# jzhoulab/orca

Hardware: AMD Instinct MI355X
Metric: Mb of sequence encoded+decoded per second (32Mb H1-ESC-shaped model, both strands, 6 levels) (higher is better)
Workload: dtype f16x2 | Encoder Conv1d stages 1-7: f16x2 = fp32 emulated as 2 x fp16 split operands, 3 MFMA products, fp32 accumulate (22 significant operand bits); Decoder / Decoder_1m Conv2d: f16x2 = fp32 emulated as 2 x fp16 split operands, 3 MFMA products, fp32 accumulate (22 significant operand bits); Encoder2; 1 GPU; H1-ESC 32Mb model forward, single random 32Mb sequence, fp32-class (f16x2 split operands on the 16-bit matrix cores, see dtype; parity vs the reference's fp32 in `parity` with --full), both strands (genomepredict-equivalent, 1 model): Encoder+Encoder2+6 Decoder+Decoder_1m per strand; sequence_bp=32000000, strands=2, levels=6, weights=synthetic seed 0, input=1 byte/base packed sequence in HBM, both strands read from it, parallelism=single GPU

## Files before the change

### include/orca_hip.h

```cpp
#ifndef ORCA_HIP_H
#define ORCA_HIP_H

#include <stddef.h>
#include <stdint.h>

#ifdef __cplusplus
extern "C" {
#endif

#define ORCA_OK 0
#define ORCA_EINVAL (-1)
#define ORCA_EHIP (-2)
#define ORCA_ENOMEM (-3)
#define ORCA_ENODEV (-4)

#define ORCA_ABI_VERSION 1

typedef struct orca_ctx orca_ctx;
typedef struct orca_net orca_net;

enum orca_net_kind {
  ORCA_NET_ENCODER = 1,
  ORCA_NET_ENCODER2 = 2,
  ORCA_NET_ENCODER3 = 3,
// ... 33 lines not shown
  int32_t ksize;
} orca_kernel_time;
int orca_ctx_set_timing(orca_ctx* ctx, int enable);
int orca_ctx_get_timing(orca_ctx* ctx, orca_kernel_time* out, int max, int* n);

int orca_ctx_launch_counts(orca_ctx* ctx, int64_t* counts4);

int orca_net_create(orca_ctx* ctx, int kind, const orca_conv_desc* convs, int n_convs,
                    int upsample_mode, orca_net** out);
int orca_net_free(orca_net* net);

#define ORCA_PRECISION_F32 0
#define ORCA_PRECISION_BF16 1
#define ORCA_PRECISION_BF16X2 2
#define ORCA_PRECISION_BF16X3 3
#define ORCA_PRECISION_F16X2 4
#define ORCA_PRECISION_F16 5
int orca_net_set_precision(orca_net* net, int precision);
#define ORCA_ENCODER_FORM_DEFAULT 0
#define ORCA_ENCODER_FORM_STORED_RESIDUAL 1
#define ORCA_ENCODER_FORM_LCONV1_ONLY 2
#define ORCA_ENCODER_FORM_TWO_CONV 3
int orca_net_set_encoder_form(orca_net* net, int form);
int orca_ctx_take_overflow(orca_ctx* ctx, int* flag);


int orca_encoder_forward(orca_ctx* ctx, orca_net* net, const float* x, int64_t sx_b, int64_t sx_c,
                         int64_t sx_l, int B, int64_t L, int64_t bin_lo, int64_t bin_hi, float* out,
                         int64_t so_b, int64_t so_c, int64_t chunk_bp);

int orca_pack_sequence(orca_ctx* ctx, const float* x, int64_t sx_c, int64_t sx_l, int64_t L, uint8_t* codes_out, int* packable);
int orca_encoder_forward_codes(orca_ctx* ctx, orca_net* net, const uint8_t* codes, int64_t sc_b, int reverse, int B, int64_t L,
                               int64_t bin_lo, int64_t bin_hi, float* out, int64_t so_b, int64_t so_c, int64_t chunk_bp);
int orca_encoder_forward_codes_window(orca_ctx* ctx, orca_net* net, const uint8_t* codes, int64_t sc_b, int64_t win_origin,
                                      int64_t win_len, int reverse, int B, int64_t L, int64_t bin_lo, int64_t bin_hi,
                                      float* out, int64_t so_b, int64_t so_c, int64_t chunk_bp);
int orca_encoder_forward_2bit(orca_ctx* ctx, orca_net* net, const uint8_t* two, const uint8_t* nmask, int64_t start, int reverse, int64_t L,
                              int64_t bin_lo, int64_t bin_hi, float* out, int64_t so_c, int64_t chunk_bp);

int64_t orca_p16_plane_units(int64_t n);
int orca_encoder_stage3_planes(orca_ctx* ctx, orca_net* net, const uint8_t* codes, int64_t L, int reverse, float* planes, int64_t plane_units);
int orca_p16_pool5_into(orca_ctx* ctx, const float* src, int64_t src_units, int64_t src_pos0, float* dst, int64_t dst_units, int64_t dst_pos0, int64_t count);
int orca_encoder_front_snippet(orca_ctx* ctx, orca_net* net, const uint8_t* codes, int64_t L, int reverse, int64_t base0, int64_t nbases, int64_t skip,
                               int64_t count, float* dst, int64_t dst_units, int64_t dst_pos0);
int orca_encoder_back(orca_ctx* ctx, orca_net* net, const float* s4, int64_t s4_units, int64_t n4, float* out, int64_t so_c);
int orca_encoder_stage4_rows(orca_ctx* ctx, orca_net* net, const float* s4, int64_t s4_units, int64_t n4, float* rows);
// ... 71 lines not shown
#define ORCA_COMM_ID_BYTES 128
int orca_comm_unique_id(void* id128_host);
int orca_comm_init_rank(orca_ctx* ctx, int nranks, int rank, const void* id128_host, orca_comm** out);
int orca_comm_destroy(orca_comm* comm);
int orca_allgather(orca_ctx* ctx, orca_comm* comm, const float* send, float* recv, size_t count);

int orca_pointwise1d_forward(orca_ctx* ctx, const float* w_dev, const float* bias_dev, int cout, int cin, const float* x,
                             int64_t x_bs, int64_t ldx, float* y, int64_t y_bs, int64_t ldy, int B, int64_t n, int act);

int orca_conv1d_forward(orca_ctx* ctx, const orca_conv_desc* conv, const float* x, int64_t x_bs, int64_t ldx,
                        float* y, int64_t y_bs, int64_t ldy, const float* r1, const float* r2, int B, int64_t n,
                        int relu, int tile);
int orca_conv1d_nlc_forward(orca_ctx* ctx, const orca_conv_desc* conv, int precision, const float* x, float* y,
                            const float* r1, int B, int64_t n, int relu);
int orca_conv1d_p16_forward(orca_ctx* ctx, const orca_conv_desc* conv, const float* x, float* y, const float* r1,
                            int64_t n, int relu, int out_mode);
int orca_conv1d_b16_forward(orca_ctx* ctx, const orca_conv_desc* conv, const float* x, float* y, const float* r1,
                            int64_t n, int relu, int out_mode);
int orca_conv2d_forward(orca_ctx* ctx, const orca_conv_desc* conv, const float* x, float* y, const float* r,
                        int B, int n, int relu);
int orca_conv2d_m16_forward(orca_ctx* ctx, const orca_conv_desc* conv, int precision, const float* x, float* y,
                            const float* r, int B, int n, int relu);
int orca_conv2d_dblock_forward(orca_ctx* ctx, const orca_conv_desc* convs, int precision, const float* x, float* y, int B, int n);
int orca_maxpool1d_forward(orca_ctx* ctx, const float* x, int64_t ldx, float* y, int64_t ldy, int64_t rows,
                           int64_t n_out, int k);

#ifdef __cplusplus
}
#endif
#endif
```

### orca_amd/_lib.py

```python
import ctypes
import os
from ctypes import POINTER, c_char_p, c_int, c_int32, c_int64, c_size_t, c_void_p

_HERE = os.path.dirname(os.path.abspath(__file__))
LIB_PATH = os.path.join(_HERE, "csrc", "liborca_hip.so")

ORCA_NET_ENCODER, ORCA_NET_ENCODER2, ORCA_NET_ENCODER3, ORCA_NET_DECODER, ORCA_NET_DECODER_1M, ORCA_NET_ENCODER2B = 1, 2, 3, 4, 5, 6
ORCA_UPSAMPLE_NEAREST, ORCA_UPSAMPLE_BILINEAR = 0, 1
PRECISIONS = {"f32": 0, "bf16": 1, "bf16x2": 2, "bf16x3": 3, "f16x2": 4, "f16": 5}
ENCODER_FORMS = {"default": 0, "stored_residual": 1, "lconv1_only": 2, "two_conv": 3}


class OrcaHipError(RuntimeError):
    pass


class ConvDesc(ctypes.Structure):
    _fields_ = [("weight_host", c_void_p), ("bias_host", c_void_p), ("cout", c_int32), ("cin", c_int32),
                ("ksize", c_int32), ("dilation", c_int32)]


class KernelTime(ctypes.Structure):
    _fields_ = [("cout", c_int32), ("cin", c_int32), ("tile", c_int32), ("batch", c_int32), ("n", c_int64),
                ("ms", ctypes.c_float), ("ksize", c_int32)]


SIGNATURES = {
    "orca_abi_version": (c_int, []),
    "orca_last_error": (c_char_p, []),
    "orca_device_count": (c_int, []),
    "orca_ctx_create": (c_int, [c_int, c_void_p, POINTER(c_void_p)]),
    "orca_ctx_destroy": (c_int, [c_void_p]),
    "orca_ctx_set_stream": (c_int, [c_void_p, c_void_p]),
    "orca_ctx_workspace_bytes": (c_int, [c_void_p, POINTER(c_size_t)]),
    "orca_ctx_release_workspace": (c_int, [c_void_p]),
    "orca_ctx_take_overflow": (c_int, [c_void_p, POINTER(c_int)]),
    "orca_ctx_set_timing": (c_int, [c_void_p, c_int]),
    "orca_ctx_get_timing": (c_int, [c_void_p, POINTER(KernelTime), c_int, POINTER(c_int)]),
    "orca_ctx_launch_counts": (c_int, [c_void_p, POINTER(ctypes.c_int64)]),
    "orca_net_create": (c_int, [c_void_p, c_int, POINTER(ConvDesc), c_int, c_int, POINTER(c_void_p)]),
    "orca_net_free": (c_int, [c_void_p]),
    "orca_net_set_precision": (c_int, [c_void_p, c_int]),
    "orca_net_set_encoder_form": (c_int, [c_void_p, c_int]),
    "orca_encoder_forward": (c_int, [c_void_p, c_void_p, c_void_p, c_int64, c_int64, c_int64, c_int, c_int64, c_int64,
                                     c_int64, c_void_p, c_int64, c_int64, c_int64]),
    "orca_p16_plane_units": (c_int64, [c_int64]),
    "orca_encoder_stage3_planes": (c_int, [c_void_p, c_void_p, c_void_p, c_int64, c_int, c_void_p, c_int64]),
    "orca_p16_pool5_into": (c_int, [c_void_p, c_void_p, c_int64, c_int64, c_void_p, c_int64, c_int64, c_int64]),
    "orca_encoder_front_snippet": (c_int, [c_void_p, c_void_p, c_void_p, c_int64, c_int, c_int64, c_int64, c_int64, c_int64, c_void_p, c_int64, c_int64]),
    "orca_encoder_back": (c_int, [c_void_p, c_void_p, c_void_p, c_int64, c_int64, c_void_p, c_int64]),
    "orca_encoder_stage4_rows": (c_int, [c_void_p, c_void_p, c_void_p, c_int64, c_int64, c_void_p]),
    "orca_rows_pool5_into": (c_int, [c_void_p, c_void_p, c_int64, c_int64, c_void_p, c_int64, c_int64, c_int64]),
    "orca_encoder_front4_snippet": (c_int, [c_void_p, c_void_p, c_void_p, c_int64, c_int, c_int64, c_int64, c_int64, c_int64, c_void_p, c_int64, c_int64]),
    "orca_encoder_front4_ranges": (c_int, [c_void_p, c_void_p, c_void_p, c_int64, c_int, c_int, POINTER(ctypes.c_int64), c_void_p, c_int64]),
    "orca_encoder_back5": (c_int, [c_void_p, c_void_p, c_void_p, c_int64, c_void_p, c_int64]),
    "orca_screen_edit_codes": (c_int, [c_void_p, c_void_p, c_int64, c_void_p, c_int, c_void_p, c_int64, c_void_p, c_int64]),
    "orca_screen_splice_rows": (c_int, [c_void_p, c_void_p, c_int64, c_void_p, c_int64, c_void_p, c_int, c_void_p]),
    "orca_encoder_back5_batch": (c_int, [c_void_p, c_void_p, c_void_p, c_int, c_int64, c_void_p, c_int64, c_int64]),
    "orca_screen_scores": (c_int, [c_void_p, c_void_p, c_int64, c_void_p, c_int, c_int, c_void_p, c_void_p, c_void_p]),
    "orca_screen_edit_codes_multi": (c_int, [c_void_p, c_void_p, c_int64, c_void_p, c_void_p, c_int, c_void_p, c_void_p, c_int64, c_void_p, c_int64, c_void_p,
                                             c_int64]),
    "orca_screen_splice_rows_multi": (c_int, [c_void_p, c_void_p, c_int64, c_void_p, c_int64, c_void_p, c_void_p, c_int64, c_void_p, c_void_p, c_int, c_void_p]),
    "orca_screen_region_scores": (c_int, [c_void_p, c_void_p, c_int64, c_void_p, c_int, c_int, c_void_p, c_void_p, c_int, c_void_p, c_void_p]),
    "orca_screen_assemble_codes": (c_int, [c_void_p, c_void_p, c_int64, c_void_p, c_void_p, c_int, c_void_p, c_void_p, c_int64, c_void_p, c_int64, c_void_p,
                                           c_int64]),
    "orca_screen_gather_rows": (c_int, [c_void_p, c_void_p, c_int64, c_void_p, c_int64, c_void_p, c_void_p, c_void_p, c_int, c_void_p, c_void_p, c_int64, c_void_p,
# ... 14 lines not shown
    "orca_decoder_forward_rows": (c_int, [c_void_p, c_void_p, POINTER(c_void_p), c_int64, c_int64, POINTER(c_void_p), c_int64, c_int64, c_int64,
                                          POINTER(c_void_p), c_int64, c_int64, c_int64, c_int, c_int, c_void_p, c_int]),
    "orca_decoder1m_forward_rows": (c_int, [c_void_p, c_void_p, POINTER(c_void_p), c_int64, c_int64, c_int, c_int, c_void_p, c_int]),
    "orca_net_num_targets": (c_int, [c_void_p, POINTER(c_int)]),
    "orca_decoder1m_forward": (c_int, [c_void_p, c_void_p, c_void_p, c_int64, c_int64, c_int64, c_int, c_int, c_void_p, c_int]),
    "orca_decoder_probe": (c_int, [c_void_p, c_void_p, c_void_p, c_int64, c_int64, c_int64, c_void_p, c_int64, c_int64, c_int64, c_int64, c_void_p,
                                   c_int64, c_int64, c_int64, c_int64, c_int, c_int, c_int, c_int, c_void_p]),
    "orca_strand_merge": (c_int, [c_void_p, c_void_p, c_void_p, c_void_p, c_int]),
    "orca_block_mean_f64": (c_int, [c_void_p, c_void_p, c_int64, c_int64, c_int64, c_int, c_int, c_void_p, c_void_p, c_int]),
    "orca_adaptive_coarsegrain": (c_int, [c_void_p, c_void_p, c_void_p, c_int64, c_int, ctypes.c_float, c_int, c_int, c_void_p, c_int64]),
    "orca_genome_unpack_2bit": (c_int, [c_void_p, c_void_p, c_void_p, c_int64, c_int64, c_void_p]),
    "orca_comm_unique_id": (c_int, [c_void_p]),
    "orca_comm_init_rank": (c_int, [c_void_p, c_int, c_int, c_void_p, POINTER(c_void_p)]),
    "orca_comm_destroy": (c_int, [c_void_p]),
    "orca_allgather": (c_int, [c_void_p, c_void_p, c_void_p, c_void_p, c_size_t]),
    "orca_conv1d_forward": (c_int, [c_void_p, POINTER(ConvDesc), c_void_p, c_int64, c_int64, c_void_p, c_int64, c_int64,
                                    c_void_p, c_void_p, c_int, c_int64, c_int, c_int]),
    "orca_conv1d_nlc_forward": (c_int, [c_void_p, POINTER(ConvDesc), c_int, c_void_p, c_void_p, c_void_p, c_int, c_int64, c_int]),
    "orca_conv1d_p16_forward": (c_int, [c_void_p, POINTER(ConvDesc), c_void_p, c_void_p, c_void_p, c_int64, c_int, c_int]),
    "orca_conv1d_b16_forward": (c_int, [c_void_p, POINTER(ConvDesc), c_void_p, c_void_p, c_void_p, c_int64, c_int, c_int]),
    "orca_conv2d_forward": (c_int, [c_void_p, POINTER(ConvDesc), c_void_p, c_void_p, c_void_p, c_int, c_int, c_int]),
    "orca_conv2d_m16_forward": (c_int, [c_void_p, POINTER(ConvDesc), c_int, c_void_p, c_void_p, c_void_p, c_int, c_int, c_int]),
    "orca_conv2d_dblock_forward": (c_int, [c_void_p, POINTER(ConvDesc), c_int, c_void_p, c_void_p, c_int, c_int]),
    "orca_maxpool1d_forward": (c_int, [c_void_p, c_void_p, c_int64, c_void_p, c_int64, c_int64, c_int64, c_int]),
    "orca_pointwise1d_forward": (c_int, [c_void_p, c_void_p, c_void_p, c_int, c_int, c_void_p, c_int64, c_int64, c_void_p, c_int64,
                                          c_int64, c_int, c_int64, c_int]),
}

_lib = None


def load():
    global _lib
    if _lib is not None:
        return _lib
    if not os.path.exists(LIB_PATH):
        raise OrcaHipError(
            f"{LIB_PATH} not found: the HIP extension is not built. Run `make -C orca_amd/csrc` "
            "(or `python -c 'import __graft_entry__ as g; g.build()'`). There is no CPU fallback.")
    import torch
    lib = ctypes.CDLL(LIB_PATH)
    for name, (res, args) in SIGNATURES.items():
        fn = getattr(lib, name)
        fn.restype = res
        fn.argtypes = args
    if lib.orca_abi_version() != 1:
# ... 10 lines not shown
```

### orca_amd/csrc/conv2d_dblock.h

```cpp
#pragma once
#include "conv2d_m16.h"

struct DBlockArgs {
  f32x4* cur;
  const void* w[4];
  const float* bias[4];
  long bs;
  int H, W, dil;
  unsigned* flag;
};

#ifndef DBLOCK_STORE_WT
#define DBLOCK_STORE_WT 0
#endif
__device__ __forceinline__ void db_store_unit(u32x4_t* p, const u32x4_t& v) {
#if DBLOCK_STORE_WT
  m16_store_unit(p, v);
#else
  *p = v;
#endif
}

template <int NS, int DT, int ABL = 0>
__global__ __launch_bounds__(512, NS == 1 ? 4 : 2) void conv2d_dblock_kernel(DBlockArgs a) {
// ... 213 lines not shown
        unit_.x = h0_; unit_.y = h1_; unit_.z = l0_; unit_.w = l1_;
        if (pvalid) db_store_unit(reinterpret_cast<u32x4_t*>(cur) + m16_plane(h * 4 + q, g, NS, H) + poff, unit_);
      }
    if (pvalid && vmax > 65504.f) overflow = true;
  } else {
#pragma unroll
    for (int h = 0; h < 2; ++h)
#pragma unroll
      for (int qp = 0; qp < 2; ++qp) {
        const f32x4 v0 = acc4(h, 2 * qp, 128 + h * 32, true) + get_A(h * 4 + 2 * qp);
        const f32x4 v1 = acc4(h, 2 * qp + 1, 128 + h * 32, true) + get_A(h * 4 + 2 * qp + 1);
        if (DT == 1) vmax = p16_vmax3_abs(p16_vmax3_abs(p16_vmax3_abs(p16_vmax3_abs(vmax, v0.x, v0.y), v0.z, v0.w), v1.x, v1.y), v1.z, v1.w);
        unsigned a0_ = m16_pk2<DT>(v0.x, v0.y), a1_ = m16_pk2<DT>(v0.z, v0.w), b0_ = m16_pk2<DT>(v1.x, v1.y), b1_ = m16_pk2<DT>(v1.z, v1.w);
        p16_swap32(a0_, b0_);
        p16_swap32(a1_, b1_);
        u32x4_t unit_;
        unit_.x = a0_; unit_.y = a1_; unit_.z = b0_; unit_.w = b1_;
        if (pvalid) db_store_unit(reinterpret_cast<u32x4_t*>(cur) + m16_plane(h * 4 + 2 * qp + g, 0, NS, H) + poff, unit_);
      }
    if (DT == 1 && pvalid && vmax > 65504.f) overflow = true;
  }
  if (DT == 1 && overflow && a.flag) *a.flag = 1u;
}
```

### orca_amd/csrc/orca_core.hip

```cpp
#include "orca_internal.h"

static thread_local std::string g_err;

int fail(int code, const char* fmt, ...) {
  char buf[1024];
  va_list ap;
  va_start(ap, fmt);
  vsnprintf(buf, sizeof buf, fmt, ap);
  va_end(ap);
  g_err = buf;
  return code;
}

int ws_ensure(orca_ctx* ctx, size_t bytes) {
  ctx->ws_off = 0;
  if (ctx->ws_used && ctx->ws_stream != ctx->stream) HIPCHECK(hipStreamSynchronize(ctx->ws_stream));
  ctx->ws_stream = ctx->stream;
  ctx->ws_used = true;
  if (bytes <= ctx->ws_bytes) return ORCA_OK;
  const size_t step = bytes >= (size_t(1) << 30) ? (size_t(1) << 30) : (size_t(64) << 20);
  bytes = (bytes + step - 1) / step * step;
  if (ctx->ws) {
    HIPCHECK(hipStreamSynchronize(ctx->stream));
    HIPCHECK(hipFree(ctx->ws));
// ... 517 lines not shown
  *out = net;
  return ORCA_OK;
}

extern "C" int orca_net_set_precision(orca_net* net, int precision) {
  if (!net) return fail(ORCA_EINVAL, "net is NULL");
  if (precision < ORCA_PRECISION_F32 || precision > ORCA_PRECISION_F16) return fail(ORCA_EINVAL, "unknown precision %d", precision);
  const bool dec = net->kind == ORCA_NET_DECODER || net->kind == ORCA_NET_DECODER_1M;
  const bool unet = net->kind == ORCA_NET_ENCODER2 || net->kind == ORCA_NET_ENCODER3 || net->kind == ORCA_NET_ENCODER2B;
  if (precision != ORCA_PRECISION_F32 && !(((net->kind == ORCA_NET_ENCODER || unet) && precision != ORCA_PRECISION_F16) ||
                                           (dec && (precision == ORCA_PRECISION_F16X2 || precision == ORCA_PRECISION_BF16 || precision == ORCA_PRECISION_F16))))
    return fail(ORCA_EINVAL, "precision %d is not implemented for net kind %d", precision, net->kind);
  net->precision = precision;
  return ORCA_OK;
}

extern "C" int orca_net_set_encoder_form(orca_net* net, int form) {
  if (!net || net->kind != ORCA_NET_ENCODER) return fail(ORCA_EINVAL, "orca_net_set_encoder_form: not an Encoder net");
  if (form < ORCA_ENCODER_FORM_DEFAULT || form > ORCA_ENCODER_FORM_TWO_CONV) return fail(ORCA_EINVAL, "orca_net_set_encoder_form: form %d unknown", form);
  net->enc_form = form;
  return ORCA_OK;
}

extern "C" int orca_net_free(orca_net* net) {
  if (!net) return ORCA_OK;
  if (net->ctx) (void)hipSetDevice(net->ctx->device);
  for (auto& L : net->convs) free_layer(L);
  if (net->d_first_w) (void)hipFree(net->d_first_w);
  if (net->d_first_w16) (void)hipFree(net->d_first_w16);
  if (net->d_first_tab) (void)hipFree(net->d_first_tab);
  if (net->d_sep) (void)hipFree(net->d_sep);
  if (net->d_l1_w16) (void)hipFree(net->d_l1_w16);
  if (net->d_l1_bias) (void)hipFree(net->d_l1_bias);
  if (net->d_c1a_w16) (void)hipFree(net->d_c1a_w16);
  if (net->d_c1a_bias) (void)hipFree(net->d_c1a_bias);
  if (net->d_l1_f32) (void)hipFree(net->d_l1_f32);
  if (net->d_c1a_f32) (void)hipFree(net->d_c1a_f32);
  if (net->d_l1_bias32) (void)hipFree(net->d_l1_bias32);
  if (net->d_c1a_bias32) (void)hipFree(net->d_c1a_bias32);
  for (auto& L : net->comp) free_layer(L);
  delete net;
  return ORCA_OK;
}


extern "C" int orca_net_num_targets(orca_net* net, int* num_2d) {
// ... 6 lines not shown
```

### orca_amd/csrc/orca_decoder.hip

```cpp
#include "orca_internal.h"

#include "conv2d_m16.h"
#include "conv2d_m16q.h"
#include "conv2d_dblock.h"
#include "misc_kernels.h"
#include "coarsegrain.h"

int launch_conv2d(orca_ctx* ctx, const ConvLayer& L, const float* x, long x_bs, float* y, long y_bs,
                         const float* r, long r_bs, int B, int n, int relu) {
  if (L.ksize != 3) return fail(ORCA_EINVAL, "launch_conv2d on a non-3x3 layer");
  Conv2dArgs a;
  a.x = x; a.w = L.d_w; a.bias = L.d_bias; a.y = y; a.r = r;
  a.x_bs = x_bs; a.y_bs = y_bs; a.r_bs = r_bs; a.H = n; a.W = n; a.dil = L.dil; a.nchunks = L.nchunks; a.relu = relu;
  dim3 grid((unsigned)n, (unsigned)B);
  if (L.cout == 64) hipLaunchKernelGGL((conv2d_3x3_kernel<64>), grid, dim3(512), 0, ctx->stream, a);
  else hipLaunchKernelGGL((conv2d_3x3_kernel<32>), grid, dim3(512), 0, ctx->stream, a);
  LAUNCHCHECK("conv2d_3x3_kernel");
  return ORCA_OK;
}

int launch_conv2d_m16(orca_ctx* ctx, const ConvLayer& L, const f32x4* x, long x_bs, int x_oct, f32x4* y, long y_bs, int y_oct,
                             const f32x4* r, long r_bs, int B, int n, int relu, int mode, int chunk0, int nchunks_,
                             const float* tab, long tab_bs) {
  const bool bf16 = mode == 1;
// ... 147 lines not shown
        C2(L[7], Bf, sz64, 8, Df, sz64, 8, Cf, sz64, 1);
      } else {
        C2(pairs[0], A, szA, oA, T, sz32, 4, nullptr, 0, 0);
        C2(pairs[1], T, sz32, 4, Cf, sz64, 8, nullptr, 0, 0);
        C2(pairs[2], Cf, sz64, 8, T, sz32, 4, nullptr, 0, 1);
        C2(pairs[3], T, sz32, 4, Df, sz64, 8, Cf, sz64, 1);
      }
    } else {
      pairs = L; npairs = 19;
      C2(pairs[0], IN, szIN, oIN, T, sz32, 4, nullptr, 0, 0);
      C2(pairs[1], T, sz32, 4, Cf, sz64, 8, nullptr, 0, 0);
      C2(pairs[2], Cf, sz64, 8, T, sz32, 4, nullptr, 0, 1);
      C2(pairs[3], T, sz32, 4, Df, sz64, 8, Cf, sz64, 1);
    }
    f32x4* cur = Df;
    f32x4* oth = Cf;
    for (int i = 1; i < npairs; ++i) {
      PROBE(3 + i - 1, cur, sz64);
      const ConvLayer* p = pairs + 4 * i;
      const int dil = p[0].dil;
      if (dil >= 16) {
        if (!(dil == 16 || dil == 32 || dil == 64) || p[1].dil != dil || p[2].dil != dil || p[3].dil != dil)
          return fail(ORCA_EINVAL, "decoder block %d: dilation %d unsupported", i, dil);
        DBlockArgs da;
        da.cur = cur; da.bs = sz64; da.H = n; da.W = n; da.dil = dil; da.flag = ctx->d_flag;
        for (int k = 0; k < 4; ++k) {
          if (!bf16 && !p[k].f16_ok) return fail(ORCA_EINVAL, "layer weights exceed the fp16 range");
          da.w[k] = bf16 ? p[k].d_wb16p : p[k].d_wf16;
          da.bias[k] = p[k].d_bias;
        }
        hipLaunchKernelGGL((conv2d_dblock_kernel<NS, DT>), dim3(256, (unsigned)nb), dim3(512), 0, ctx->stream, da);
        LAUNCHCHECK("conv2d_dblock_kernel");
        continue;
      }
      C2(p[0], cur, sz64, 8, T, sz32, 4, nullptr, 0, 0);
      C2(p[1], T, sz32, 4, oth, sz64, 8, cur, sz64, 0);
      C2(p[2], oth, sz64, 8, T, sz32, 4, nullptr, 0, 1);
      C2(p[3], T, sz32, 4, cur, sz64, 8, oth, sz64, 1);
    }
#undef C2
    PROBE(3 + npairs - 1, cur, sz64);
#undef PROBE
    const ConvLayer& fa = net->convs[net->convs.size() - 2];
    const ConvLayer& fb = net->convs[net->convs.size() - 1];
    FinalArgs fa_;
    fa_.cur = reinterpret_cast<const float*>(cur); fa_.w1 = fa.d_w; fa_.b1 = fa.d_bias; fa_.w2 = fb.d_w; fa_.b2 = fb.d_bias; fa_.out = out + (size_t)b0 * nt2 * n * n;
// ... 218 lines not shown
```

### orca_amd/csrc/orca_internal.h

```cpp
#pragma once
#include <hip/hip_runtime.h>

#include <cstdarg>
#include <cstdint>
#include <cstdio>
#include <cstdlib>
#include <cstring>
#include <string>
#include <vector>

#include "conv_kernels.h"
#include "orca_hip.h"

int fail(int code, const char* fmt, ...) __attribute__((format(printf, 2, 3)));

#define HIPCHECK(expr)                                                                          \
  do {                                                                                          \
    hipError_t _e = (expr);                                                                     \
    if (_e != hipSuccess) return fail(ORCA_EHIP, "%s failed: %s (%s:%d)", #expr, hipGetErrorString(_e), __FILE__, __LINE__); \
  } while (0)

#define LAUNCHCHECK(name)                                                                        \
  do {                                                                                          \
    hipError_t _e = hipGetLastError();                                                          \
// ... 38 lines not shown
  return rc;
}

#ifndef ORCA_MAX_TARGETS
#define ORCA_MAX_TARGETS 8
#endif
#define ORCA_EDGE_SLAB (40 * 128)

struct ConvLayer {
  int cin = 0, cout = 0, ksize = 0, dil = 1;
  int kc = 8, nchunks = 0;
  float* d_w = nullptr;
  float* d_bias = nullptr;
  void* d_wb16 = nullptr;
  void* d_wf16 = nullptr;
  void* d_wb16p = nullptr;
  bool f16_ok = true;
};

struct orca_net {
  orca_ctx* ctx = nullptr;
  int kind = 0;
  int precision = ORCA_PRECISION_F32;
  int enc_form = ORCA_ENCODER_FORM_DEFAULT;
  float* d_first_w = nullptr;
  void* d_first_w16 = nullptr;
  float* d_first_tab = nullptr;
  int upsample_mode = ORCA_UPSAMPLE_BILINEAR;
  int num_2d = 1;
  float* d_sep = nullptr;
  void* d_l1_w16 = nullptr;
  float* d_l1_bias = nullptr;
  void* d_c1a_w16 = nullptr;
  float* d_c1a_bias = nullptr;
  float* d_l1_f32 = nullptr;
  float* d_c1a_f32 = nullptr;
  float* d_l1_bias32 = nullptr;
  float* d_c1a_bias32 = nullptr;
  ConvLayer comp[3];
  std::vector<ConvLayer> convs;
};

int make_layer(const orca_conv_desc& d, ConvLayer* out);
int make_layer17(int cin, int cout, const std::vector<double>& w17, const std::vector<double>& b17, ConvLayer* out);
void compose_pair(const orca_conv_desc& c1, const orca_conv_desc& c2, std::vector<double>* w17, std::vector<double>* b17);
void free_layer(ConvLayer& L);
// ... 50 lines not shown
```

### orca_amd/csrc/orca_test_entries.hip

```cpp
#include "orca_internal.h"

#include "conv_p16.h"
#include "conv2d_m16.h"
#include "conv2d_dblock.h"
#include "misc_kernels.h"

extern "C" int orca_conv1d_forward(orca_ctx* ctx, const orca_conv_desc* conv, const float* x, int64_t x_bs, int64_t ldx, float* y,
                                   int64_t y_bs, int64_t ldy, const float* r1, const float* r2, int B, int64_t n, int relu,
                                   int tile) {
  if (!ctx || !conv || !x || !y) return fail(ORCA_EINVAL, "orca_conv1d_forward: NULL argument");
  HIPCHECK(hipSetDevice(ctx->device));
  ConvLayer L;
  ORCA_TRY(make_layer(*conv, &L));
  int rc = launch_conv1d(ctx, L, x, x_bs, ldx, y, y_bs, ldy, r1, r2, B, n, relu, tile);
  (void)hipStreamSynchronize(ctx->stream);
  free_layer(L);
  return rc;
}

extern "C" int orca_conv1d_nlc_forward(orca_ctx* ctx, const orca_conv_desc* conv, int precision, const float* x, float* y,
                                       const float* r1, int B, int64_t n, int relu) {
  if (!ctx || !conv || !x || !y) return fail(ORCA_EINVAL, "orca_conv1d_nlc_forward: NULL argument");
  if (precision < ORCA_PRECISION_BF16 || precision > ORCA_PRECISION_F16X2) return fail(ORCA_EINVAL, "precision %d unsupported here", precision);
  HIPCHECK(hipSetDevice(ctx->device));
// ... 160 lines not shown
  if (!(d == 16 || d == 32 || d == 64)) return fail(ORCA_EINVAL, "orca_conv2d_dblock_forward: dilation %d (16, 32 or 64)", d);
  for (int k = 0; k < 4; ++k) {
    const int cin = k & 1 ? 32 : 64, cout = k & 1 ? 64 : 32;
    if (convs[k].ksize != 3 || convs[k].cin != cin || convs[k].cout != cout || convs[k].dilation != d)
      return fail(ORCA_EINVAL, "orca_conv2d_dblock_forward: conv %d must be 3x3, %d -> %d, dilation %d", k, cin, cout, d);
  }
  HIPCHECK(hipSetDevice(ctx->device));
  ConvLayer L[4];
  int rc = ORCA_OK;
  for (int k = 0; k < 4 && rc == ORCA_OK; ++k) {
    rc = make_layer(convs[k], &L[k]);
    if (rc == ORCA_OK && precision != ORCA_PRECISION_BF16 && !L[k].f16_ok) rc = fail(ORCA_EINVAL, "layer weights exceed the fp16 range");
  }
  if (rc == ORCA_OK) {
    if (precision == ORCA_PRECISION_F16X2) rc = conv2d_dblock_test<2, 1>(ctx, L, x, y, B, n);
    else if (precision == ORCA_PRECISION_BF16) rc = conv2d_dblock_test<1, 0>(ctx, L, x, y, B, n);
    else rc = conv2d_dblock_test<1, 1>(ctx, L, x, y, B, n);
  }
  (void)hipStreamSynchronize(ctx->stream);
  for (int k = 0; k < 4; ++k) free_layer(L[k]);
  return rc;
}

extern "C" int orca_pointwise1d_forward(orca_ctx* ctx, const float* w_dev, const float* bias_dev, int cout, int cin, const float* x,
                                        int64_t x_bs, int64_t ldx, float* y, int64_t y_bs, int64_t ldy, int B, int64_t n, int act) {
  if (!ctx || !w_dev || !bias_dev || !x || !y) return fail(ORCA_EINVAL, "orca_pointwise1d_forward: NULL argument");
  if (cout <= 0 || cin <= 0 || B <= 0 || n < 0 || act < 0 || act > 2) return fail(ORCA_EINVAL, "orca_pointwise1d_forward: bad shape / activation");
  if (n == 0) return ORCA_OK;
  HIPCHECK(hipSetDevice(ctx->device));
  dim3 grid((unsigned)((n + 255) / 256), (unsigned)cout, (unsigned)B);
  hipLaunchKernelGGL(pointwise1d_kernel, grid, dim3(256), 0, ctx->stream, w_dev, bias_dev, cin, x, (long)x_bs, (long)ldx, y, (long)y_bs,
                     (long)ldy, (long)n, act);
  LAUNCHCHECK("pointwise1d_kernel");
  return ORCA_OK;
}

extern "C" int orca_maxpool1d_forward(orca_ctx* ctx, const float* x, int64_t ldx, float* y, int64_t ldy, int64_t rows,
                                      int64_t n_out, int k) {
  if (!ctx || !x || !y) return fail(ORCA_EINVAL, "orca_maxpool1d_forward: NULL argument");
  HIPCHECK(hipSetDevice(ctx->device));
  return launch_pool(ctx, x, ldx, y, ldy, rows, n_out, k);
}
```

### orca_amd/engine.py

```python
import ctypes
import threading
import weakref

import numpy as np
import torch

from . import _lib
from ._lib import ConvDesc, OrcaHipError, check

BN_EPS = 1e-5


_tls = threading.local()


class Context:
    def __init__(self, device_index):
        lib = _lib.load()
        self.device_index = device_index
        self.handle = ctypes.c_void_p()
        stream = torch.cuda.current_stream(device_index).cuda_stream
        check(lib.orca_ctx_create(device_index, ctypes.c_void_p(stream), ctypes.byref(self.handle)), "orca_ctx_create")
        self._finalizer = weakref.finalize(self, lib.orca_ctx_destroy, self.handle)

# ... 233 lines not shown
        lib = _lib.load()
        self.ctx, self.kind = ctx, kind
        self.handle = ctypes.c_void_p()
        descs = make_descs(convs)
        check(lib.orca_net_create(ctx.handle, kind, descs, len(convs), upsample_mode, ctypes.byref(self.handle)), "orca_net_create")
        self._finalizer = weakref.finalize(self, lib.orca_net_free, self.handle)

    def num_targets(self):
        if getattr(self, "_num_targets", None) is None:
            t = ctypes.c_int(0)
            check(_lib.load().orca_net_num_targets(self.handle, ctypes.byref(t)), "orca_net_num_targets")
            self._num_targets = int(t.value)
        return self._num_targets

    def set_precision(self, name):
        if name not in _lib.PRECISIONS:
            raise ValueError(f"precision must be one of {sorted(_lib.PRECISIONS)}, got {name!r}")
        check(_lib.load().orca_net_set_precision(self.handle, _lib.PRECISIONS[name]), "orca_net_set_precision")

    def set_encoder_form(self, name):
        if name not in _lib.ENCODER_FORMS:
            raise ValueError(f"form must be one of {sorted(_lib.ENCODER_FORMS)}, got {name!r}")
        check(_lib.load().orca_net_set_encoder_form(self.handle, _lib.ENCODER_FORMS[name]), "orca_net_set_encoder_form")


def _f32_cuda(t, name):
    if not isinstance(t, torch.Tensor):
        raise TypeError(f"{name} must be a torch.Tensor")
    if not t.is_cuda:
        raise OrcaHipError(f"{name} is on '{t.device}': orca_amd has no CPU path (move it to the MI355X with .cuda())")
    if t.dtype != torch.float32:
        t = t.float()
    return t


def _p(t):
    return ctypes.c_void_p(t.data_ptr())


def encoder_num_bins(L):
    return int(_lib.load().orca_encoder_num_bins(int(L)))


def encoder_forward(net, x, bin_lo=0, bin_hi=0, chunk_bp=0, out=None):
    x = _f32_cuda(x, "x")
    if x.dim() != 3 or x.shape[1] != 4:
# ... 621 lines not shown
    r = r.contiguous() if r is not None else None
    check(_lib.load().orca_conv2d_m16_forward(ctx.handle, d, _lib.PRECISIONS[precision], _p(x), _p(y), _p(r) if r is not None else None, B, n,
                                              1 if relu else 0), "orca_conv2d_m16_forward")
    return y


def conv2d_dblock(x, convs, dilation, precision="f16x2"):
    x = _f32_cuda(x, "x").contiguous()
    B, _, n, _ = x.shape
    layers = []
    for w, b in convs:
        w = np.ascontiguousarray(w, dtype=np.float32)
        layers.append({"w": w, "b": np.ascontiguousarray(b, dtype=np.float32), "cout": w.shape[0], "cin": w.shape[1], "k": w.shape[2],
                       "dil": int(dilation)})
    if len(layers) != 4:
        raise ValueError("conv2d_dblock: four convs (lm.a, lm.b, m.a, m.b)")
    d = make_descs(layers)
    y = torch.empty_like(x)
    ctx = get_context(x.device)
    check(_lib.load().orca_conv2d_dblock_forward(ctx.handle, d, _lib.PRECISIONS[precision], _p(x), _p(y), B, n), "orca_conv2d_dblock_forward")
    return y


def maxpool1d(x, k):
    x = _f32_cuda(x, "x").contiguous()
    B, C, n = x.shape
    y = torch.empty((B, C, n // k), dtype=torch.float32, device=x.device)
    ctx = get_context(x.device)
    check(_lib.load().orca_maxpool1d_forward(ctx.handle, _p(x), n, _p(y), n // k, B * C, n // k, k), "orca_maxpool1d_forward")
    return y


def pointwise1d(x, w_dev, b_dev, act="none"):
    x = _f32_cuda(x, "x").contiguous()
    B, cin, n = x.shape
    cout = w_dev.shape[0]
    if tuple(w_dev.shape) != (cout, cin) or not w_dev.is_cuda or not w_dev.is_contiguous():
        raise ValueError("w_dev must be a contiguous [cout,cin] ROCm tensor")
    y = torch.empty((B, cout, n), dtype=torch.float32, device=x.device)
    ctx = get_context(x.device)
    check(_lib.load().orca_pointwise1d_forward(ctx.handle, _p(w_dev), _p(b_dev), cout, cin, _p(x), cin * n, n, _p(y), cout * n, n, B, n,
                                               {"none": 0, "relu": 1, "sigmoid": 2}[act]), "orca_pointwise1d_forward")
    return y
```

Before: 1006 Mb/s.

## Fuse dilation 16/32/64 decoder blocks into one LDS-resident run kernel

Adds a kernel that runs three consecutive dilated decoder residual blocks (dilations 16, 32, 64) in one launch. The activation tile stays in shared memory between blocks, and the next block's weights are prefetched through a rotating three-slot buffer. This is meant to cut two of the three global round-trips of the 64-channel map and the launch boundaries between blocks. It is on by default for f16x2 decoders. The tile pixel mapping must cover all three dilations, which adds complexity and correctness risk.

New measurement: 1016 Mb/s, median of 6. +1.0%, better.

```diff
diff --git a/include/orca_hip.h b/include/orca_hip.h
--- a/include/orca_hip.h
+++ b/include/orca_hip.h
@@ -79,6 +79,7 @@
 #define ORCA_ENCODER_FORM_LCONV1_ONLY 2
 #define ORCA_ENCODER_FORM_TWO_CONV 3
 int orca_net_set_encoder_form(orca_net* net, int form);
+int orca_net_set_decoder_block_runs(orca_net* net, int on);
 int orca_ctx_take_overflow(orca_ctx* ctx, int* flag);
 
 
@@ -196,6 +197,8 @@
 int orca_conv2d_m16_forward(orca_ctx* ctx, const orca_conv_desc* conv, int precision, const float* x, float* y,
                             const float* r, int B, int n, int relu);
 int orca_conv2d_dblock_forward(orca_ctx* ctx, const orca_conv_desc* convs, int precision, const float* x, float* y, int B, int n);
+int orca_conv2d_dblock_run_forward(orca_ctx* ctx, const orca_conv_desc* convs, int nblk, int precision, const float* x, float* y, int B, int n,
+                                   int fused);
 int orca_maxpool1d_forward(orca_ctx* ctx, const float* x, int64_t ldx, float* y, int64_t ldy, int64_t rows,
                            int64_t n_out, int k);
 
diff --git a/orca_amd/_lib.py b/orca_amd/_lib.py
--- a/orca_amd/_lib.py
+++ b/orca_amd/_lib.py
@@ -42,6 +42,7 @@
     "orca_net_free": (c_int, [c_void_p]),
     "orca_net_set_precision": (c_int, [c_void_p, c_int]),
     "orca_net_set_encoder_form": (c_int, [c_void_p, c_int]),
+    "orca_net_set_decoder_block_runs": (c_int, [c_void_p, c_int]),
     "orca_encoder_forward": (c_int, [c_void_p, c_void_p, c_void_p, c_int64, c_int64, c_int64, c_int, c_int64, c_int64,
                                      c_int64, c_void_p, c_int64, c_int64, c_int64]),
     "orca_p16_plane_units": (c_int64, [c_int64]),
@@ -102,6 +103,7 @@
     "orca_conv2d_forward": (c_int, [c_void_p, POINTER(ConvDesc), c_void_p, c_void_p, c_void_p, c_int, c_int, c_int]),
     "orca_conv2d_m16_forward": (c_int, [c_void_p, POINTER(ConvDesc), c_int, c_void_p, c_void_p, c_void_p, c_int, c_int, c_int]),
     "orca_conv2d_dblock_forward": (c_int, [c_void_p, POINTER(ConvDesc), c_int, c_void_p, c_void_p, c_int, c_int]),
+    "orca_conv2d_dblock_run_forward": (c_int, [c_void_p, POINTER(ConvDesc), c_int, c_int, c_void_p, c_void_p, c_int, c_int, c_int]),
     "orca_maxpool1d_forward": (c_int, [c_void_p, c_void_p, c_int64, c_void_p, c_int64, c_int64, c_int64, c_int]),
     "orca_pointwise1d_forward": (c_int, [c_void_p, c_void_p, c_void_p, c_int, c_int, c_void_p, c_int64, c_int64, c_void_p, c_int64,
                                           c_int64, c_int, c_int64, c_int]),
diff --git a/orca_amd/csrc/conv2d_dblock.h b/orca_amd/csrc/conv2d_dblock.h
--- a/orca_amd/csrc/conv2d_dblock.h
+++ b/orca_amd/csrc/conv2d_dblock.h
@@ -259,3 +259,258 @@
   }
   if (DT == 1 && overflow && a.flag) *a.flag = 1u;
 }
+
+struct DBlockRunArgs {
+  f32x4* cur;
+  long bs;
+  int H, W, dil0, nblk;
+  const void* w[12];
+  const float* bias[12];
+  unsigned* flag;
+};
+
+template <int NS, int DT, int ABL = 0>
+__global__ __launch_bounds__(512, 2) void conv2d_dblock_run_kernel(DBlockRunArgs a) {
+  static_assert(NS == 2 && DT == 1, "f16x2 only (see above)");
+  constexpr int WNS = 2;
+  constexpr int NT = 512, PXW = 256 + 16;
+  constexpr int AU = NS * 8 * PXW, BU = NS * 4 * PXW;
+  constexpr int WP = NS * 9 * 2 * 32;
+  constexpr int WIT = (WP + NT - 1) / NT;
+  constexpr int EXTRA = (WP - (WIT - 1) * NT + 63) / 64;
+  constexpr int MAXBLK = 3;
+  __shared__ f32x4 smem[AU + BU + 3 * WP + 48 * MAXBLK];
+  f32x4* const As = smem;
+  f32x4* const Bs = smem + AU;
+  f32x4* const Ws = smem + AU + BU;
+  float* const bias_s = reinterpret_cast<float*>(smem + AU + BU + 3 * WP);
+
+  const int tid = threadIdx.x, lane = tid & 63;
+  const int wave = __builtin_amdgcn_readfirstlane(tid >> 6);
+  const int l31 = lane & 31, g = lane >> 5;
+  const int d = a.dil0, H = a.H, W = a.W, nblk = a.nblk;
+  const int ld = 31 - __builtin_clz(d);
+  const int lS = 8 - ld, S = 1 << lS;
+  const int lG = 2 * ld - 8, G = 1 << lG;
+  f32x4* const cur = a.cur + (long)blockIdx.y * a.bs;
+
+  int bx = (int)blockIdx.x;
+  {
+    const int xcd = bx & 7, t = bx >> 3;
+    if (G == 1) { const int run = xcd * 4 + (t >> 3); bx = (run >> 1) * 16 + (run & 1) * 8 + (t & 7); }
+    else if (G == 4) { const int pair = xcd * 16 + (t >> 1); bx = pair * 2 + (t & 1); }
+  }
+  auto pix = [&](int p, int& row, int& col, int& r, int& c) {
+    const int sid = (bx << lG) + (p >> (2 * lS)), q = p & ((1 << (2 * lS)) - 1);
+    r = q >> lS; c = q & (S - 1);
+    row = (sid >> ld) + (r << ld);
+    col = (sid & (d - 1)) + (c << ld);
+  };
+  {
+    const int sid0 = bx << lG;
+    if ((sid0 >> ld) >= H || (sid0 & (d - 1)) >= W) return;
+  }
+
+  if (tid < NS * 8 * 16) As[(tid >> 4) * PXW + 256 + (tid & 15)] = (f32x4)(0.f);
+  if (tid >= 256 && tid < 256 + NS * 4 * 16) Bs[((tid - 256) >> 4) * PXW + 256 + (tid & 15)] = (f32x4)(0.f);
+  __syncthreads();
+  if (wave == 0 && lane < 48) {
+#pragma unroll
+    for (int b = 0; b < MAXBLK; ++b)
+      if (b < nblk) {
+        const float *b0 = a.bias[4 * b], *b1 = a.bias[4 * b + 1], *b2 = a.bias[4 * b + 2], *b3 = a.bias[4 * b + 3];
+        const float* src = lane < 8 ? b0 + 4 * lane : (lane < 24 ? b1 + 4 * (lane - 8) : (lane < 32 ? b2 + 4 * (lane - 24) : b3 + 4 * (lane - 32)));
+        p16_glds16(reinterpret_cast<const f32x4*>(src), smem + AU + BU + 3 * WP + 48 * b);
+      }
+  }
+
+  auto issue_piece = [&](const void* wl, int i, int slot) {
+    const int L = i >> 2, j = i & 3;
+    const bool wide = L & 1;
+    const int k = wide ? (j & 1) : j, h = wide ? (j >> 1) : 0, cout = wide ? 64 : 32;
+    f32x4* dst = Ws + slot;
+#pragma unroll
+    for (int it = 0; it < WIT; ++it) {
+      const int u = tid + it * NT;
+      const int grp = u >> 5, co = u & 31;
+      if (u < WP) p16_glds16(reinterpret_cast<const f32x4*>(wl) + ((long)k * (WNS * 9 * 2) + grp) * cout + h * 32 + co, dst + it * NT + wave * 64);
+    }
+  };
+  int ro0 = 0, ro1 = WP, ro2 = 2 * WP;
+  {
+    int row, col, r_, c_;
+    pix(tid & 255, row, col, r_, c_);
+    const bool ok = row < H && col < W;
+    const long off = ok ? (long)row * M16_PX + col : 255;
+#pragma unroll
+    for (int k = 0; k < 4; ++k) {
+#pragma unroll
+      for (int s_ = 0; s_ < NS; ++s_) {
+        const int plane = s_ * 8 + 2 * k + (wave >> 2);
+        if (!(ABL & 4)) p16_glds16(cur + m16_plane(plane & 7, s_, NS, H) + off, As + plane * PXW + (wave & 3) * 64);
+      }
+      if (k < 3) issue_piece(a.w[0], k, k * WP);
+    }
+  }
+
+  const int p = wave * 32 + l31;
+  int prow, pcol, pr, pc;
+  pix(p, prow, pcol, pr, pc);
+  const bool pvalid = prow < H && pcol < W;
+  const long poff = (long)prow * M16_PX + pcol;
+
+  f32x16 acc[2];
+  const unsigned as_lds = p16_lds_addr(As), bs_lds = p16_lds_addr(Bs), ws_lds = p16_lds_addr(Ws + g * 32 + l31);
+  bool overflow = false;
+  auto put = [&](f32x4* Xs, int XG, int oct, f32x4 v) {
+    if (!pvalid) v = (f32x4)(0.f);
+    u32x2 sp[NS];
+    split4<NS, DT>(v, sp, overflow);
+#pragma unroll
+    for (int s = 0; s < NS; ++s) *reinterpret_cast<u32x2*>(reinterpret_cast<char*>(Xs + (s * XG + oct) * PXW + p) + 8 * g) = sp[s];
+  };
+  auto get_A = [&](int oct) -> f32x4 {
+    float f[4] = {0.f, 0.f, 0.f, 0.f};
+#pragma unroll
+    for (int s = 0; s < NS; ++s) {
+      const u32x2 u = *reinterpret_cast<const u32x2*>(reinterpret_cast<const char*>(As + (s * 8 + oct) * PXW + p) + 8 * g);
+      float a0, a1, a2, a3;
+      m16_pair<DT>(u.x, a0, a1);
+      m16_pair<DT>(u.y, a2, a3);
+      f[0] += a0; f[1] += a1; f[2] += a2; f[3] += a3;
+    }
+    f32x4 r;
+    r.x = f[0]; r.y = f[1]; r.z = f[2]; r.w = f[3];
+    return r;
+  };
+  auto acc4 = [&](int h, int q, const float* bl, bool relu) -> f32x4 {
+    const f32x4 b = *reinterpret_cast<const f32x4*>(bl + 8 * q + 4 * g);
+    f32x4 v;
+    v.x = acc[h][4 * q + 0] + b.x; v.y = acc[h][4 * q + 1] + b.y; v.z = acc[h][4 * q + 2] + b.z; v.w = acc[h][4 * q + 3] + b.w;
+    if (relu) { v.x = p16_vmax(v.x, 0.f); v.y = p16_vmax(v.y, 0.f); v.z = p16_vmax(v.z, 0.f); v.w = p16_vmax(v.w, 0.f); }
+    return v;
+  };
+  auto zero_acc = [&]() {
+#pragma unroll
+    for (int h = 0; h < 2; ++h)
+#pragma unroll
+      for (int r = 0; r < 16; ++r) acc[h][r] = 0.f;
+  };
+  auto wait_next = [&]() {
+    if (wave < EXTRA) asm volatile("s_waitcnt vmcnt(%0)" ::"n"(WIT) : "memory");
+    else asm volatile("s_waitcnt vmcnt(%0)" ::"n"(WIT - 1) : "memory");
+  };
+
+#define DBR_READ(buf_, t_)                                                                                        \
+  _Pragma("unroll") for (int s = 0; s < NS; ++s) {                                                                \
+    xv[buf_][s] = p16_lds_read16(xrow + nb16[t_], s * XG * PXW * 16);                                             \
+    wv[buf_][s] = p16_lds_read16(wrow, ((s * 9 + (t_)) * 2) * 32 * 16);                                           \
+  }
+#define DBR_LAYER(LY, XLDS, XG_, WIDE)                                                                            \
+  {                                                                                                               \
+    constexpr int XG = XG_;                                                                                       \
+    _Pragma("unroll") for (int j = 0; j < 4; ++j) {                                                               \
+      constexpr bool wide_ = WIDE;                                                                                \
+      const int piece = 4 * (LY) + j;                                                                             \
+      const int k = wide_ ? (j & 1) : j;                                                                          \
+      const int h = wide_ ? (j >> 1) : 0;                                                                         \
+      if (piece <= 2 && first) {                                                                                  \
+        if (piece == 0) {                                                                                         \
+          if (wave < EXTRA) asm volatile("s_waitcnt vmcnt(%0)" ::"n"(3 * NS + 2 * WIT) : "memory");              \
+          else asm volatile("s_waitcnt vmcnt(%0)" ::"n"(3 * NS + 2 * (WIT - 1)) : "memory");                     \
+        } else if (piece == 1) {                                                                                  \
+          if (wave < EXTRA) asm volatile("s_waitcnt vmcnt(%0)" ::"n"(2 * NS + WIT) : "memory");                  \
+          else asm volatile("s_waitcnt vmcnt(%0)" ::"n"(2 * NS + WIT - 1) : "memory");                           \
+        } else {                                                                                                  \
+          if (wave < EXTRA) asm volatile("s_waitcnt vmcnt(%0)" ::"n"(NS + WIT) : "memory");                      \
+          else asm volatile("s_waitcnt vmcnt(%0)" ::"n"(NS + WIT - 1) : "memory");                               \
+        }                                                                                                         \
+      } else if (piece == 15 && last) asm volatile("s_waitcnt vmcnt(0)" ::: "memory");                            \
+      else wait_next();                                                                                           \
+      asm volatile("s_waitcnt lgkmcnt(0)\n\ts_barrier" ::: "memory");                                             \
+      if (!(ABL & 2)) {                                                                                           \
+        const int slot2 = (piece + 2) % 3 == 0 ? ro0 : ((piece + 2) % 3 == 1 ? ro1 : ro2);                        \
+        if (piece == 0) { if (!first) issue_piece(wb[0], 2, slot2); }                                             \
+        else if (piece >= 14) { if (!last) issue_piece(wb[4], piece - 14, slot2); }                               \
+        else issue_piece(wb[(piece + 2) >> 2], piece + 2, slot2);                                                 \
+      }                                                                                                           \
+      const unsigned wrow = ws_lds + (unsigned)((piece % 3 == 0 ? ro0 : (piece % 3 == 1 ? ro1 : ro2)) * 16);     \
+      const unsigned xrow = (XLDS) + (unsigned)((2 * k + g) * PXW * 16);                                          \
+      f16x8 xv[2][NS], wv[2][NS];                                                                                 \
+      DBR_READ(0, 0);                                                                                             \
+      _Pragma("unroll") for (int t = 0; t < 9; ++t) {                                                             \
+        const int fb = t & 1;                                                                                     \
+        if (t + 1 < 9) { DBR_READ(fb ^ 1, t + 1); m16_wait<2 * NS, NS>(xv[fb], wv[fb]); }                         \
+        else m16_wait<0, NS>(xv[fb], wv[fb]);                                                                     \
+        typedef typename Op16<DT>::vec V_;                                                                        \
+        if constexpr ((ABL & 1) != 0) { asm volatile("" ::"v"(xv[fb][0]), "v"(wv[fb][0])); }                     \
+        else {                                                                                                    \
+          acc[h] = Op16<DT>::mfma(__builtin_bit_cast(V_, wv[fb][0]), __builtin_bit_cast(V_, xv[fb][NS - 1]), acc[h]); \
+          acc[h] = Op16<DT>::mfma(__builtin_bit_cast(V_, wv[fb][NS - 1]), __builtin_bit_cast(V_, xv[fb][0]), acc[h]); \
+          acc[h] = Op16<DT>::mfma(__builtin_bit_cast(V_, wv[fb][0]), __builtin_bit_cast(V_, xv[fb][0]), acc[h]); \
+        }                                                                                                         \
+        __builtin_amdgcn_sched_barrier(0);                                                                        \
+      }                                                                                                           \
+    }                                                                                                             \
+  }
+
+  float vmax = 0.f;
+#pragma unroll 1
+  for (int b = 0; b < nblk; ++b) {
+    const bool first = b == 0, last = b + 1 == nblk;
+    const void* wb[5];
+#pragma unroll
+    for (int q = 0; q < 5; ++q) wb[q] = a.w[4 * b + (q < 4 || !last ? q : 0)];
+    const float* const bl = bias_s + 192 * b;
+    unsigned nb16[9];
+#pragma unroll
+    for (int t = 0; t < 9; ++t) {
+      const int dy = (t / 3 - 1) * (1 << b), dx = (t % 3 - 1) * (1 << b);
+      const bool in = (unsigned)(pr + dy) < (unsigned)S && (unsigned)(pc + dx) < (unsigned)S;
+      nb16[t] = (in ? (unsigned)(p + dy * S + dx) : 256u + ((unsigned)(p + dy * S + dx) & 15u)) * 16u;
+    }
+    zero_acc();
+    DBR_LAYER(0, as_lds, 8, false);
+#pragma unroll
+    for (int q = 0; q < 4; ++q) put(Bs, 4, q, acc4(0, q, bl, false));
+    zero_acc();
+    DBR_LAYER(1, bs_lds, 4, true);
+#pragma unroll
+    for (int h = 0; h < 2; ++h)
+#pragma unroll
+      for (int q = 0; q < 4; ++q) put(As, 8, h * 4 + q, acc4(h, q, bl + 32 + h * 32, false) + get_A(h * 4 + q));
+    zero_acc();
+    DBR_LAYER(2, as_lds, 8, false);
+#pragma unroll
+    for (int q = 0; q < 4; ++q) put(Bs, 4, q, acc4(0, q, bl + 96, true));
+    zero_acc();
+    DBR_LAYER(3, bs_lds, 4, true);
+#pragma unroll
+    for (int h = 0; h < 2; ++h)
+#pragma unroll
+      for (int q = 0; q < 4; ++q) {
+        f32x4 v = acc4(h, q, bl + 128 + h * 32, true) + get_A(h * 4 + q);
+        vmax = p16_vmax3_abs(p16_vmax3_abs(vmax, v.x, v.y), v.z, v.w);
+        if (!pvalid) v = (f32x4)(0.f);
+        unsigned h0_, h1_, l0_, l1_;
+        p16_split_hl(v, h0_, h1_, l0_, l1_);
+        if (last) {
+          p16_swap32(h0_, l0_);
+          p16_swap32(h1_, l1_);
+          u32x4_t unit_;
+          unit_.x = h0_; unit_.y = h1_; unit_.z = l0_; unit_.w = l1_;
+          if (pvalid) db_store_unit(reinterpret_cast<u32x4_t*>(cur) + m16_plane(h * 4 + q, g, NS, H) + poff, unit_);
+        } else {
+          u32x2 hi_, lo_;
+          hi_.x = h0_; hi_.y = h1_; lo_.x = l0_; lo_.y = l1_;
+          *reinterpret_cast<u32x2*>(reinterpret_cast<char*>(As + (h * 4 + q) * PXW + p) + 8 * g) = hi_;
+          *reinterpret_cast<u32x2*>(reinterpret_cast<char*>(As + (8 + h * 4 + q) * PXW + p) + 8 * g) = lo_;
+        }
+      }
+    { const int t_ = ro0; ro0 = ro1; ro1 = ro2; ro2 = t_; }
+  }
+#undef DBR_LAYER
+#undef DBR_READ
+  if (pvalid && vmax > 65504.f) overflow = true;
+  if (overflow && a.flag) *a.flag = 1u;
+}
diff --git a/orca_amd/csrc/orca_core.hip b/orca_amd/csrc/orca_core.hip
--- a/orca_amd/csrc/orca_core.hip
+++ b/orca_amd/csrc/orca_core.hip
@@ -563,6 +563,12 @@
   return ORCA_OK;
 }
 
+extern "C" int orca_net_set_decoder_block_runs(orca_net* net, int on) {
+  if (!net || (net->kind != ORCA_NET_DECODER && net->kind != ORCA_NET_DECODER_1M)) return fail(ORCA_EINVAL, "orca_net_set_decoder_block_runs: not a Decoder net");
+  net->dec_block_runs = on ? 1 : 0;
+  return ORCA_OK;
+}
+
 extern "C" int orca_net_free(orca_net* net) {
   if (!net) return ORCA_OK;
   if (net->ctx) (void)hipSetDevice(net->ctx->device);
diff --git a/orca_amd/csrc/orca_decoder.hip b/orca_amd/csrc/orca_decoder.hip
--- a/orca_amd/csrc/orca_decoder.hip
+++ b/orca_amd/csrc/orca_decoder.hip
@@ -193,6 +193,23 @@
       if (dil >= 16) {
         if (!(dil == 16 || dil == 32 || dil == 64) || p[1].dil != dil || p[2].dil != dil || p[3].dil != dil)
           return fail(ORCA_EINVAL, "decoder block %d: dilation %d unsupported", i, dil);
+        if constexpr (NS == 2 && DT == 1) {
+          bool is_run = net->dec_block_runs && dil == 16 && i + 2 < npairs && !(probe && (probe->stage == 3 + i || probe->stage == 3 + i + 1));
+          for (int k = 0; is_run && k < 8; ++k) is_run = p[4 + k].dil == (k < 4 ? 32 : 64);
+          if (is_run) {
+            DBlockRunArgs ra{};
+            ra.cur = cur; ra.bs = sz64; ra.H = n; ra.W = n; ra.dil0 = 16; ra.nblk = 3; ra.flag = ctx->d_flag;
+            for (int k = 0; k < 12; ++k) {
+              if (!p[k].f16_ok) return fail(ORCA_EINVAL, "layer weights exceed the fp16 range");
+              ra.w[k] = p[k].d_wf16;
+              ra.bias[k] = p[k].d_bias;
+            }
+            hipLaunchKernelGGL((conv2d_dblock_run_kernel<2, 1>), dim3(256, (unsigned)nb), dim3(512), 0, ctx->stream, ra);
+            LAUNCHCHECK("conv2d_dblock_run_kernel");
+            i += 2;
+            continue;
+          }
+        }
         DBlockArgs da;
         da.cur = cur; da.bs = sz64; da.H = n; da.W = n; da.dil = dil; da.flag = ctx->d_flag;
         for (int k = 0; k < 4; ++k) {
diff --git a/orca_amd/csrc/orca_internal.h b/orca_amd/csrc/orca_internal.h
--- a/orca_amd/csrc/orca_internal.h
+++ b/orca_amd/csrc/orca_internal.h
@@ -84,6 +84,7 @@
   orca_ctx* ctx = nullptr;
   int kind = 0;
   int precision = ORCA_PRECISION_F32;
+  int dec_block_runs = 1;
   int enc_form = ORCA_ENCODER_FORM_DEFAULT;
   float* d_first_w = nullptr;
   void* d_first_w16 = nullptr;
diff --git a/orca_amd/csrc/orca_test_entries.hip b/orca_amd/csrc/orca_test_entries.hip
--- a/orca_amd/csrc/orca_test_entries.hip
+++ b/orca_amd/csrc/orca_test_entries.hip
@@ -206,6 +206,55 @@
   return rc;
 }
 
+extern "C" int orca_conv2d_dblock_run_forward(orca_ctx* ctx, const orca_conv_desc* convs, int nblk, int precision, const float* x, float* y, int B,
+                                              int n, int fused) {
+  if (!ctx || !convs || !x || !y) return fail(ORCA_EINVAL, "orca_conv2d_dblock_run_forward: NULL argument");
+  if (n <= 0 || n > ORCA_LDW || B <= 0 || B > 65535) return fail(ORCA_EINVAL, "orca_conv2d_dblock_run_forward: map size %d / batch %d unsupported", n, B);
+  if (precision != ORCA_PRECISION_F16X2) return fail(ORCA_EINVAL, "orca_conv2d_dblock_run_forward: precision %d has no run kernel (f16x2 only)", precision);
+  if (nblk != 2 && nblk != 3) return fail(ORCA_EINVAL, "orca_conv2d_dblock_run_forward: %d blocks (2 or 3)", nblk);
+  const int d0 = convs[0].dilation;
+  if (!(d0 == 16 || d0 == 32) || (d0 << (nblk - 1)) > 64) return fail(ORCA_EINVAL, "orca_conv2d_dblock_run_forward: %d blocks from dilation %d (16, 32 (, 64) or 32, 64)", nblk, d0);
+  for (int k = 0; k < 4 * nblk; ++k) {
+    const int cin = k & 1 ? 32 : 64, cout = k & 1 ? 64 : 32, d = d0 << (k >> 2);
+    if (convs[k].ksize != 3 || convs[k].cin != cin || convs[k].cout != cout || convs[k].dilation != d)
+      return fail(ORCA_EINVAL, "orca_conv2d_dblock_run_forward: conv %d must be 3x3, %d -> %d, dilation %d", k, cin, cout, d);
+  }
+  HIPCHECK(hipSetDevice(ctx->device));
+  ConvLayer L[12];
+  int rc = ORCA_OK, made = 0;
+  for (; made < 4 * nblk && rc == ORCA_OK; ++made) {
+    rc = make_layer(convs[made], &L[made]);
+    if (rc == ORCA_OK && !L[made].f16_ok) rc = fail(ORCA_EINVAL, "layer weights exceed the fp16 range");
+  }
+  const size_t sz64 = (size_t)2 * n * ORCA_LDW * 8;
+  if (rc == ORCA_OK) rc = ws_ensure(ctx, ru256(B * sz64 * 16));
+  if (rc == ORCA_OK) {
+    f32x4* cur = reinterpret_cast<f32x4*>(ws_take(ctx, B * sz64 * 4));
+    hipStream_t s = ctx->stream;
+    for (int b = 0; b < B; ++b)
+      hipLaunchKernelGGL((nchw_to_m16_kernel<2, 1>), dim3((unsigned)n), dim3(ORCA_LDW), 0, s, x + (size_t)b * 64 * n * n, 64, n, cur + b * sz64, 8);
+    if (fused) {
+      DBlockRunArgs ra{};
+      ra.cur = cur; ra.bs = (long)sz64; ra.H = n; ra.W = n; ra.dil0 = d0; ra.nblk = nblk; ra.flag = ctx->d_flag;
+      for (int k = 0; k < 4 * nblk; ++k) { ra.w[k] = L[k].d_wf16; ra.bias[k] = L[k].d_bias; }
+      hipLaunchKernelGGL((conv2d_dblock_run_kernel<2, 1>), dim3(256, (unsigned)B), dim3(512), 0, s, ra);
+    } else {
+      for (int blk = 0; blk < nblk; ++blk) {
+        DBlockArgs da;
+        da.cur = cur; da.bs = (long)sz64; da.H = n; da.W = n; da.dil = d0 << blk; da.flag = ctx->d_flag;
+        for (int k = 0; k < 4; ++k) { da.w[k] = L[4 * blk + k].d_wf16; da.bias[k] = L[4 * blk + k].d_bias; }
+        hipLaunchKernelGGL((conv2d_dblock_kernel<2, 1>), dim3(256, (unsigned)B), dim3(512), 0, s, da);
+      }
+    }
+    for (int b = 0; b < B; ++b)
+      hipLaunchKernelGGL((m16_to_nchw_kernel<2, 1>), dim3((unsigned)n), dim3(ORCA_LDW), 0, s, cur + b * sz64, 64, n, y + (size_t)b * 64 * n * n);
+    if (hipGetLastError() != hipSuccess) rc = fail(ORCA_EHIP, "conv2d_dblock_run test path: launch failed");
+  }
+  (void)hipStreamSynchronize(ctx->stream);
+  for (int k = 0; k < made; ++k) free_layer(L[k]);
+  return rc;
+}
+
 extern "C" int orca_pointwise1d_forward(orca_ctx* ctx, const float* w_dev, const float* bias_dev, int cout, int cin, const float* x,
                                         int64_t x_bs, int64_t ldx, float* y, int64_t y_bs, int64_t ldy, int B, int64_t n, int act) {
   if (!ctx || !w_dev || !bias_dev || !x || !y) return fail(ORCA_EINVAL, "orca_pointwise1d_forward: NULL argument");
diff --git a/orca_amd/engine.py b/orca_amd/engine.py
--- a/orca_amd/engine.py
+++ b/orca_amd/engine.py
@@ -279,6 +279,9 @@
         if name not in _lib.ENCODER_FORMS:
             raise ValueError(f"form must be one of {sorted(_lib.ENCODER_FORMS)}, got {name!r}")
         check(_lib.load().orca_net_set_encoder_form(self.handle, _lib.ENCODER_FORMS[name]), "orca_net_set_encoder_form")
+
+    def set_decoder_block_runs(self, on):
+        check(_lib.load().orca_net_set_decoder_block_runs(self.handle, 1 if on else 0), "orca_net_set_decoder_block_runs")
 
 
 def _f32_cuda(t, name):
@@ -946,6 +949,24 @@
     return y
 
 
+def conv2d_dblock_run(x, convs, d0, fused=True, precision="f16x2"):
+    x = _f32_cuda(x, "x").contiguous()
+    B, _, n, _ = x.shape
+    if len(convs) not in (8, 12):
+        raise ValueError("conv2d_dblock_run: four convs (lm.a, lm.b, m.a, m.b) for each of 2 or 3 blocks")
+    layers = []
+    for k, (w, b) in enumerate(convs):
+        w = np.ascontiguousarray(w, dtype=np.float32)
+        layers.append({"w": w, "b": np.ascontiguousarray(b, dtype=np.float32), "cout": w.shape[0], "cin": w.shape[1], "k": w.shape[2],
+                       "dil": int(d0) << (k // 4)})
+    d = make_descs(layers)
+    y = torch.empty_like(x)
+    ctx = get_context(x.device)
+    check(_lib.load().orca_conv2d_dblock_run_forward(ctx.handle, d, len(convs) // 4, _lib.PRECISIONS[precision], _p(x), _p(y), B, n,
+                                                     1 if fused else 0), "orca_conv2d_dblock_run_forward")
+    return y
+
+
 def maxpool1d(x, k):
     x = _f32_cuda(x, "x").contiguous()
     B, C, n = x.shape
```
